# wizzard0/llama2.ts

Measured on AMD Instinct MI355X. Metric: decode tokens/sec + achieved HBM GB/s (% peak), 1 GPU, higher is better.
Workload: dtype f64; 1 GPU; llama2_7b batch-1 greedy decode, 49 tokens from BOS (-t 0 -s 1 -n 49); parallelism=single

## Files before the change

### include/llama2_hip.h

```cpp
#ifndef LLAMA2_HIP_H
#define LLAMA2_HIP_H
#include <stddef.h>
#include <stdint.h>

#ifdef __cplusplus
extern "C" {
#endif

#define L2_ABI_VERSION 5

enum {
  L2_OK = 0,
  L2_E_ARG = -1,
  L2_E_CONFIG = -2,
  L2_E_HIP = -3,
  L2_E_STATE = -4,
  L2_E_NOGPU = -5,
  L2_E_COMM = -6
};

enum {
  L2_T_TOKEN_EMBEDDING = 0,
  L2_T_RMS_ATT = 1,
  L2_T_WQ = 2,
// ... 17 lines not shown
};

enum {
  L2_OPT_EXACT_ATTENTION = 1,
  L2_OPT_USE_GRAPH = 2,
  L2_OPT_KEEP_STATE = 3,
  L2_OPT_PACKED_MIB = 4,
  L2_OPT_WEIGHT_MIB = 5,
  L2_OPT_SAMPLED_TOKENS = 6,
  L2_OPT_SAMPLED_SERIAL = 7,
  L2_OPT_AQL_QUEUE = 8,
  L2_OPT_PREFILL_F32_MFMA = 9,
  L2_OPT_CHECK_POS = 10,
  L2_OPT_SEQS = 11,
  L2_OPT_BATCH_SAMPLED_TOKENS = 12,
  L2_OPT_BATCH_SAMPLED_SERIAL = 13
};

typedef struct l2_ctx l2_ctx;

int l2_abi_version(void);
int l2_device_count(void);
const char* l2_last_error(void);

int l2_create(const int32_t cfg[7], int device, l2_ctx** out);
void l2_destroy(l2_ctx* ctx);

enum { L2_F_GQA = 1, L2_F_GENERATE_ROPE = 2 };
int l2_create_ex(const int32_t cfg[7], int device, unsigned flags, l2_ctx** out);

int l2_tp_unique_id(void* id_out_128);
// ... 63 lines not shown
```

### llama2.ts_amd/csrc/attention.hip.h

```cpp
#pragma once
#include "kernels.hip.h"

namespace l2k {

struct AttnArgs {
  Mut<const float> q;
  Mut<const float> kc;
  Mut<const float> vc;
  Mut<float> att;
  Mut<float> xb;
  const int* tokpos;
  Mut<double> part;
  unsigned* counter;
  int dim, head_size, seq_len, n_heads, nsplit;
  int kv_dim, kv_mul;
  double inv_sqrt_hs;
  int exact;
  int pos_plus1;
  const unsigned long long* gran;
  unsigned* gran_ep;
  int fused_four_waves;
  int* herr;
  unsigned long long wait_ticks;
  unsigned long long* gout;
  const unsigned* gout_ep;
  unsigned long long* dbg;
};

__device__ __forceinline__ void attn_out(const AttnArgs& a, size_t idx, float v, unsigned otag) {
  if (a.gout) granule_store(a.gout + idx, v, otag);
  a.xb.st(idx, v);
}

template <int N>
__device__ __forceinline__ void granules_wait(const unsigned long long* const (&g)[N], float (&v)[N], unsigned tag, int* herr, unsigned long long wait_ticks, unsigned* dead) {
  unsigned spins = 0;
  unsigned long long t0 = 0;
  for (;;) {
    unsigned long long x[N];
#pragma unroll
// ... 77 lines not shown
  if (FUSED) {
    const unsigned tag = ftag = ld_word(const_cast<const unsigned*>(a.gran_ep) + h) + 1u;
    const unsigned long long* gq = a.gran + (size_t)h * hs + cc4;
    const bool need_k = own_pos && wave == NW - 1 && lane < hs, need_v = own_pos && tid < hs;
    const unsigned long long* const gp[7] = {gq, gq + 1, gq + 2, gq + 3,
        need_k ? a.gran + (size_t)h * hs + lane : gq, need_k ? a.gran + (size_t)a.dim + (size_t)hk * hs + lane : gq,
        need_v ? a.gran + (size_t)a.dim + a.kv_dim + (size_t)hk * hs + tid : gq};
    float gvals[7];
    granules_wait<7>(gp, gvals, tag, a.herr, a.wait_ticks, a.gran_ep + a.n_heads);
    STAMP(6);
    q4.x = gvals[0]; q4.y = gvals[1]; q4.z = gvals[2]; q4.w = gvals[3];
    gk_q = need_k ? gvals[4] : 0.0f; gk_k = need_k ? gvals[5] : 0.0f; gv = need_v ? gvals[6] : 0.0f;
  }
  const double q0 = cl ? (double)q4.x : 0.0, q1 = cl ? (double)q4.y : 0.0, q2 = cl ? (double)q4.z : 0.0, q3 = cl ? (double)q4.w : 0.0;
  const double rsq = a.inv_sqrt_hs;
  const unsigned otag = a.gout ? __hip_atomic_load(a.gout_ep, __ATOMIC_RELAXED, __HIP_MEMORY_SCOPE_AGENT) + 1u : 0u;
  double* Pw = P + (size_t)wave * NT * ATT_PS;
  STAMP(1);

  auto score_round = [&](const f4 (&buf)[NT], int rd) {
#pragma unroll
    for (int j = 0; j < NT; ++j) {
      const double s = (q0 * (double)buf[j].x + q1 * (double)buf[j].y) + (q2 * (double)buf[j].z + q3 * (double)buf[j].w);
      Pw[j * ATT_PS + lane] = s;
    }
    __builtin_amdgcn_wave_barrier();
#pragma unroll
    for (int dd = lane; dd < NT * RPT; dd += 64) {
      const int rr = dd / NT, j = dd % NT;
      const int tr = ((rd * NT + j) * NW + wave) * RPT + rr;
      const double* pp = Pw + j * ATT_PS + rr * LR;
// ... 214 lines not shown
  }
  attn_tile_dispatch<LR, 8, NT, true>(at, smem, h, sp, pos);
}

template <int XV, int R, int LR, int NW, int NT>
__global__ void __launch_bounds__(512) attn_wo_kernel(const AttnArgs at, const PhaseArgs wo, const int nattn) {
  extern __shared__ __attribute__((aligned(16))) char smem[];
  if ((int)blockIdx.x >= nattn) { phase_small_body<MODE_WO, XV, R, true>(wo, smem, (int)blockIdx.x - nattn, (int)gridDim.x - nattn); return; }
  if (NW * 64 < 512 && (int)threadIdx.x >= NW * 64) return;
  int sp = 0, h = (int)blockIdx.x;
  while (h >= at.n_heads) { h -= at.n_heads; ++sp; }
  const int pos = at.tokpos[1];
  attn_tile_dispatch<LR, NW, NT>(at, smem, h, sp, pos);
}

template <int LR, int NW, int NT>
__global__ void __launch_bounds__(64 * NW) attn_tile_kernel(const AttnArgs a) {
  extern __shared__ __attribute__((aligned(16))) char smem[];
  asm volatile("" ::"s"(a.q.addr()), "s"(a.kc.addr()), "s"(a.vc.addr()), "s"(a.att.addr()), "s"(a.xb.addr()), "s"(a.tokpos), "s"(a.part.addr()), "s"(a.counter));
  const int pos = a.tokpos[1];
  asm volatile("" ::"s"(a.dim), "s"(a.head_size), "s"(a.seq_len), "s"(a.n_heads), "s"(a.nsplit), "s"(a.kv_dim), "s"(a.kv_mul), "s"(a.inv_sqrt_hs), "s"(a.gout), "s"(a.gout_ep));
  attn_tile_dispatch<LR, NW, NT>(a, smem, blockIdx.x, blockIdx.y, pos);
}

template <int LR, int NW, int NT>
__global__ void __launch_bounds__(64 * NW) pf_attn_tile_kernel(const AttnArgs a, int pos0) {
  extern __shared__ __attribute__((aligned(16))) char smem[];
  AttnArgs b = a;
  const int p = blockIdx.y;
  b.q = a.q + (size_t)p * a.dim;
// ... 79 lines not shown
```

### llama2.ts_amd/csrc/attention_inst.hip.h

```cpp
#pragma once
#include "attention.hip.h"

#ifndef L2_ATTN_INST
#define L2_ATTN_INST extern
#endif

namespace l2k {
#define L2_AT_INST(LR, NW, NT) \
  L2_ATTN_INST template __global__ void attn_tile_kernel<LR, NW, NT>(const AttnArgs); \
  L2_ATTN_INST template __global__ void pf_attn_tile_kernel<LR, NW, NT>(const AttnArgs, int); \
  L2_ATTN_INST template __global__ void bt_attn_tile_kernel<LR, NW, NT>(const AttnArgs, const AttnRows);
L2_AT_INST(4, 4, 16) L2_AT_INST(8, 4, 16) L2_AT_INST(16, 4, 16) L2_AT_INST(32, 8, 8) L2_AT_INST(64, 4, 16)
#undef L2_AT_INST
L2_ATTN_INST template __global__ void qkv_attn_small_kernel<2, 16, 8>(const PhaseArgs, const AttnArgs, const int);
L2_ATTN_INST template __global__ void qkv_attn_small_kernel<3, 16, 8>(const PhaseArgs, const AttnArgs, const int);
L2_ATTN_INST template __global__ void qkv_attn_small_kernel<4, 16, 8>(const PhaseArgs, const AttnArgs, const int);
L2_ATTN_INST template __global__ void attn_wo_kernel<2, 2, 32, 8, 8>(const AttnArgs, const PhaseArgs, const int);
L2_ATTN_INST template __global__ void attn_wo_kernel<4, 2, 32, 8, 8>(const AttnArgs, const PhaseArgs, const int);
L2_ATTN_INST template __global__ void attn_wo_kernel<8, 2, 32, 8, 8>(const AttnArgs, const PhaseArgs, const int);
}
```

### llama2.ts_amd/csrc/ctx.hip.h

```cpp
#pragma once

static thread_local char g_err[512] = "";

static int fail(int code, const char* fmt, ...) {
  va_list ap;
  va_start(ap, fmt);
  vsnprintf(g_err, sizeof(g_err), fmt, ap);
  va_end(ap);
  return code;
}

#define HIPCHK(expr)                                                                              \
  do {                                                                                            \
    hipError_t e_ = (expr);                                                                       \
    if (e_ != hipSuccess) return fail(L2_E_HIP, "%s failed: %s (%s:%d)", #expr, hipGetErrorString(e_), __FILE__, __LINE__); \
  } while (0)

typedef struct { char internal[128]; } nccl_uid;
typedef void* nccl_comm;
struct Rccl {
  void* so = nullptr;
  int (*GetUniqueId)(nccl_uid*) = nullptr;
  int (*CommInitRank)(nccl_comm*, int, nccl_uid, int) = nullptr;
  int (*CommDestroy)(nccl_comm) = nullptr;
// ... 98 lines not shown
  int samp_mode = 0;
  std::shared_ptr<LoopGroup> loop;
  double* loop_tmp = nullptr;
  bool tp_path = false;
  bool p2p = false;
  void* p2p_base = nullptr;
  unsigned long long* p2p_epoch = nullptr;
  int* p2p_err = nullptr;
  int* p2p_err_dev = nullptr;
  P2PPeers p2p_peers = {};
  std::vector<void*> p2p_opened;
  bool p2p_peers_ready = false;
  unsigned long long* awo_gran = nullptr;
  unsigned* awo_ep = nullptr;
  int opt_awo = 1;
  TpPush* tp_push = nullptr;
  int opt_push = 1;
  bool rccl_graph = false;
  unsigned long long p2p_wait_ticks = 3000000000ull;
  int p2p_fenced = 0;
  bool solo = false;
  bool p2p_synced = false;
  bool broken = false;

  float* w[L2_T_COUNT] = {};
  size_t layer_elems[L2_T_COUNT] = {};
  int layers_of[L2_T_COUNT] = {};
  std::vector<uint8_t> uploaded[L2_T_COUNT];

  float *x = nullptr, *xb = nullptr, *xb2 = nullptr, *hb = nullptr, *hb2 = nullptr, *q = nullptr, *k = nullptr,
// ... 135 lines not shown
```

### llama2.ts_amd/csrc/kernels.hip.h

```cpp
#pragma once
#include <hip/hip_runtime.h>
#include <stdint.h>
#include <type_traits>

namespace l2k {

typedef float f4 __attribute__((ext_vector_type(4)));

enum { MODE_QKV = 0, MODE_WO = 1, MODE_W13 = 2, MODE_W2 = 3, MODE_CLS = 4 };

enum { CTR_STRIDE = 32 };

#ifdef L2_STAMPS
#define L2_NSTAMP 12
struct Stamps {
  unsigned long long t[L2_NSTAMP];
  unsigned long long* dst;
  unsigned long long* wg;
  unsigned long long rt0;
  __device__ __forceinline__ Stamps(unsigned long long* dbg, unsigned long long* dbg_wg = nullptr, int force_sel = -2, bool last_wave = false) {
    wg = (dbg_wg && threadIdx.x == (last_wave ? blockDim.x - 64 : 0) && blockIdx.y == 0 && blockIdx.x < 1024) ? dbg_wg + 2 * blockIdx.x : nullptr;
    rt0 = __builtin_readcyclecounter();
    asm volatile("s_memrealtime %0\n\ts_waitcnt lgkmcnt(0)" : "=s"(rt0));
#pragma unroll
// ... 100 lines not shown
  const struct TpPush* push;
  double inv_n;
  int rot;
  const float* wp;
  unsigned long long* amax;
  unsigned long long* gran;
  const unsigned* gran_ep;
  unsigned gran_hmagic;
  int* gin_herr;
  int* tok_out;
#ifdef L2_STAMPS
  unsigned long long* dbg;
  unsigned long long* dbg_wg;
#endif
};
static_assert(sizeof(void*) != 8 || sizeof(PhaseArgs) <= 224 + 16, "PhaseArgs: keep the kernel-argument block within four 64-byte lines");

struct TpPush { unsigned long long* gin[8]; const unsigned long long* epoch; int G, rank, n, solo; };

typedef unsigned u32x4 __attribute__((ext_vector_type(4)));
__device__ __forceinline__ void tp_push_store(unsigned long long* slot, double v, unsigned tag) {
  const unsigned long long b = (unsigned long long)__double_as_longlong(v);
  const u32x4 w = {(unsigned)b, tag, (unsigned)(b >> 32), tag};
  asm volatile("global_store_dwordx4 %0, %1, off sc0 sc1\n\ts_nop 1" ::"v"(slot), "v"(w) : "memory");
}
struct PushCtx { unsigned long long* gin = nullptr; int G = 0, rank = 0, n = 0, solo = 0; unsigned e = 0; };
__device__ __forceinline__ PushCtx tp_push_ctx(const TpPush* p, int lane) {
  PushCtx c;
  c.G = __builtin_amdgcn_readfirstlane(p->G); c.rank = __builtin_amdgcn_readfirstlane(p->rank);
  c.n = __builtin_amdgcn_readfirstlane(p->n); c.solo = __builtin_amdgcn_readfirstlane(p->solo);
  c.gin = p->gin[c.solo ? c.rank : min(lane, c.G - 1)];
// ... 910 lines not shown
```

### llama2.ts_amd/csrc/launch.hip.h

```cpp
#pragma once

struct Geo { int R, U, pre, nwaves, grid; bool vec; };

struct GeoKnobs { int n_cus, tune_U, tune_nwaves, tune_gridcap; };
static GeoKnobs geo_knobs(const l2_ctx* c) { return {c->n_cus, c->tune_U, c->tune_nwaves, c->tune_gridcap}; }

static Geo pick_geo_pure(const GeoKnobs& kb, int mode, int rows, int n) {
  Geo g;
  g.vec = (n % 4) == 0;
  const int n4 = n / 4;
  const int pair = (mode == MODE_W13) ? 2 : 1;
  g.R = 2;
  int U = 2;
  if (n4 > 128 && n4 <= 256) U = 4;
  if (mode == MODE_CLS && n4 > 128 && n4 <= 192) U = 3;
  if (kb.tune_U == 2 || kb.tune_U == 4 || (kb.tune_U == 3 && mode == MODE_CLS && n4 > 128 && n4 <= 192)) U = kb.tune_U;
  g.U = U;
  const int groups = (rows * pair + g.R - 1) / g.R;
  g.nwaves = groups >= 512 ? 4 : (groups >= 256 ? 2 : 1);
  if (kb.tune_nwaves == 1 || kb.tune_nwaves == 2 || kb.tune_nwaves == 4) g.nwaves = kb.tune_nwaves;
  if (mode == MODE_QKV && U == 4) g.nwaves = 4;
  const int cpi = 64 * U, npad4 = ((n4 + cpi - 1) / cpi) * cpi, nth = 64 * g.nwaves;
  g.pre = (npad4 <= nth) ? 1 : (npad4 <= 4 * nth ? 4 : 12);
  int grid = (groups + g.nwaves - 1) / g.nwaves;
// ... 52 lines not shown
    if (!name || aql_record(m->aql, m->aql_rec, name, g, b, (unsigned)lds, buf, off)) m->aql_rec_failed = true;
    return;
  }
  hipLaunchKernelGGL(kernel, grid, block, lds, st, a...);
}

static void pollute_behind(const l2_ctx* c, hipStream_t st) {
  PolluteArgs p;
  memset(&p, 0, sizeof(p));
  int nb = 0;
  auto add = [&](const void* b, size_t bytes) { if (b && bytes && nb < 20) { p.buf[nb] = (const float*)b; p.bytes[nb] = (unsigned)(bytes > 16384 ? 16384 : bytes); ++nb; } };
  add(c->x, (size_t)c->d * 4); add(c->xn, (size_t)c->d * 4); add(c->xb, (size_t)c->d_loc * 4); add(c->xb2, (size_t)c->d * 4);
  add(c->hb, (size_t)c->h_loc * 4); add(c->hb2, (size_t)c->h_loc * 4); add(c->q, (size_t)c->d_loc * 4); add(c->k, (size_t)c->kvd_loc * 4); add(c->v, (size_t)c->kvd_loc * 4);
  add(c->logits_loc, (size_t)c->V_loc * 4); add(c->amax, 8 * 16 * 8); add(c->attn_counter, (size_t)c->H_loc * CTR_STRIDE * 4);
  add(c->attn_part, (size_t)c->H_loc * 8 * (((size_t)c->hs + 2 + 15) & ~(size_t)15) * 8); add(c->gran, ((size_t)c->d_loc + 2 * (size_t)c->kvd_loc) * 8);
  add(c->gran_ep, (size_t)c->H_loc * 4 + 16); add(c->tokpos, 16); add(c->d_tokens, (size_t)c->S * 4); add(c->att, (size_t)c->H_loc * c->S * 4);
  p.nb = nb; p.kc = c->kc; p.vc = c->vc; p.tokpos = c->tokpos; p.sink = c->pollute_sink; p.L = c->L; p.S = c->S; p.kvd = c->kvd_loc;
  l2_launch_one(c, l1_pollute_kernel, dim3(c->n_cus * 4), dim3(256), 0, st, p);
}

template <class K, class A>
static void launch_probed(const l2_ctx* c, K kernel, dim3 grid, dim3 block, size_t lds, hipStream_t st, const A& a, bool probe) {
  l2_ctx* m = const_cast<l2_ctx*>(c);
  if (probe && m->probe_on && m->probe_used + 2 <= m->probe.size()) {
    hipEvent_t e0 = m->probe[m->probe_used], e1 = m->probe[m->probe_used + 1];
    m->probe_used += 2;
    hipExtLaunchKernelGGL(kernel, grid, block, lds, st, e0, e1, 0, a);
  } else {
    l2_launch(c, kernel, grid, block, lds, st, a);
  }
}
// ... 214 lines not shown
  PhaseArgs wo = wo_in;
  wo.gran = c->awo_gran; wo.gran_ep = c->awo_ep; wo.gin_herr = c->h_herr_dev;
  const int nattn = c->H_loc * at.nsplit, xv = (c->d_loc / 4 + 63) / 64;
  const int groups = (wo.rows + 1) / 2;
  int nwo = c->n_cus - nattn;
  if (nwo < c->n_cus / 2) nwo = c->n_cus / 2;
  if (nwo > groups) nwo = groups;
  const size_t lds_a = attn_tile_lds(c->S, at.nsplit, 8, 8), lds_w = (size_t)xv * 64 * 16, lds = lds_a > lds_w ? lds_a : lds_w;
  const dim3 grid(nattn + nwo), block(512);
#define L2_AWO(XVV) do { hipError_t e_ = lds_opt_in(&attn_wo_kernel<XVV, 2, 32, 8, 8>, lds); if (e_ != hipSuccess) return e_; \
                         l2_launch(c, attn_wo_kernel<XVV, 2, 32, 8, 8>, grid, block, lds, st, at, wo, nattn); } while (0)
  if (xv == 2) L2_AWO(2); else if (xv == 4) L2_AWO(4); else L2_AWO(8);
#undef L2_AWO
  return hipGetLastError();
}
```

### llama2.ts_amd/csrc/llama2_hip.hip

```cpp
#include "../../include/llama2_hip.h"

#include <dlfcn.h>
#include <hip/hip_runtime.h>
#include <hip/hip_ext.h>
#include <math.h>
#include <stdarg.h>
#include <stdio.h>
#include <stdlib.h>
#include <string.h>
#include <unistd.h>

#include <chrono>
#include <condition_variable>
#include <map>
#include <memory>
#include <mutex>
#include <string>
#include <type_traits>
#include <algorithm>
#include <vector>

#include "kernels.hip.h"
#include "attention_inst.hip.h"
#include "prefill.hip.h"
// ... 24 lines not shown
    if (c->aql_greedy[i]) { aql_program_free(c->aql_greedy[i]); c->aql_greedy[i] = nullptr; }
    if (c->aql_step[i]) { aql_program_free(c->aql_step[i]); c->aql_step[i] = nullptr; }
    if (i == 0 && c->aql_last) { aql_program_free(c->aql_last); c->aql_last = nullptr; }
    for (int m = 0; m < 4; ++m) if (c->aql_sample[i][m]) { aql_program_free(c->aql_sample[i][m]); c->aql_sample[i][m] = nullptr; }
  }
  if (c->aql) aql_reset(c->aql);
  for (int i = 0; i < NLEV; ++i) {
    if (c->g_step[i]) { hipGraphExecDestroy(c->g_step[i]); c->g_step[i] = nullptr; }
    if (c->g_greedy[i]) { hipGraphExecDestroy(c->g_greedy[i]); c->g_greedy[i] = nullptr; }
    for (int m = 0; m < 4; ++m) if (c->g_sample[i][m]) { hipGraphExecDestroy(c->g_sample[i][m]); c->g_sample[i][m] = nullptr; }
  }
}

static const int kSplitLevels[NLEV] = {1, 1, 8};
static bool fused_shape_ok(const l2_ctx* c);
static int split_level(const l2_ctx* c, int pos) {
  if (c->attn_splits_forced > 0 || c->opt_exact) return 0;
  const bool fusable = fused_shape_ok(c);
  int unsplit_to = (c->split_rows_set || !fusable) ? c->split_rows : 256;
  if (fusable && unsplit_to > 256) unsplit_to = 256;
  const int rows = pos + 1;
  if (rows > unsplit_to) return 2;
  return (fusable && rows > c->fuse_min_rows) ? 1 : 0;
}
static int splits_of(const l2_ctx* c, int level) { return c->attn_splits_forced > 0 ? c->attn_splits_forced : kSplitLevels[level]; }
static void set_level(l2_ctx* c, int level) {
  c->cur_splits = splits_of(c, level);
  c->cur_fused = level == 1 || (c->opt_fuse_splits && !c->opt_exact && fused_shape_ok(c));
}

extern "C" void l2_destroy(l2_ctx* c) {
  if (!c) return;
  hipSetDevice(c->device);
  if (c->stream) hipStreamSynchronize(c->stream);
  destroy_graphs(c);
  batch_free(c);
  if (c->aql) { aql_destroy(c->aql); c->aql = nullptr; }
  if (c->comm && g_rccl.CommDestroy) g_rccl.CommDestroy(c->comm);
  if (c->loop_tmp) hipFree(c->loop_tmp);
  for (void* m : c->p2p_opened) hipIpcCloseMemHandle(m);
  if (c->p2p_base) hipFree(c->p2p_base);
  if (c->p2p_epoch) hipFree(c->p2p_epoch);
  if (c->tp_push) hipFree(c->tp_push);
// ... 73 lines not shown
  c->tune_gridcap = dev_int("L2_TUNE_GRIDCAP", 0);
  c->tune_rot = dev_int("L2_TUNE_ROT", 5);
  c->opt_packed = dev_int("L2_PACKED", 1);
  c->opt_one_copy = dev_int("L2_ONE_COPY", 1);
  c->opt_graph = env_int("L2_USE_GRAPH", (G == 1 && !hook_int("L2_TP_FORCE_COMM")) ? 1 : 0);
  c->profile_sync = dev_int("L2_PROFILE_SYNC", 0);
  c->opt_aql = env_int("L2_AQL", 1);
  c->opt_pollute = hook_int("L2_DEBUG_POLLUTE");
  c->debug_fail_aql = hook_int("L2_DEBUG_FAIL_AQL_RUN");
  c->opt_pos_check = env_int("L2_CHECK_POS", 0);
  { const int f = dev_int("L2_AQL_FENCE", -1);
    c->aql_fence = dev_int("L2_AQL_ACQ", f < 0 ? 0 : f) + 4 * dev_int("L2_AQL_REL", f < 0 ? 1 : f) + 16 * dev_int("L2_AQL_TOKACQ", f < 0 ? 1 : 0); }
  c->p2p_fenced = env_int("L2_TP_FENCED", 0) ? 1 : 0;
  c->opt_push = dev_int("L2_TP_PUSH", 1) && !c->p2p_fenced;
  c->opt_awo = dev_int("L2_TP_ATTN_WO", 1);
  { const int ws = env_int("L2_TP_WAIT_S", 30); c->p2p_wait_ticks = (unsigned long long)(ws > 0 ? ws : 30) * 100000000ull; }

#define CK(expr) do { hipError_t e_ = (expr); if (e_ != hipSuccess) { int rc_ = fail(L2_E_HIP, "%s failed: %s", #expr, hipGetErrorString(e_)); l2_destroy(c); return rc_; } } while (0)
  CK(hipStreamCreateWithFlags(&c->stream, hipStreamNonBlocking));
  CK(hipEventCreate(&c->ev0));
  CK(hipEventCreate(&c->ev1));
  for (int k = 0; k < L2_T_COUNT; ++k) {
    const Slice s = tensor_slice(c, k);
    c->layers_of[k] = is_layered(k) ? L : 1;
    c->layer_elems[k] = s.rows * s.cols;
    if (k == L2_T_WCLS && c->shared) {
      if (G == 1) { c->w[k] = c->w[L2_T_TOKEN_EMBEDDING]; c->uploaded[k].assign(1, 0); continue; }
      c->w[k] = c->w[L2_T_TOKEN_EMBEDDING] + (size_t)rank * c->V_loc * d;
      c->uploaded[k].assign(1, 0);
      continue;
    }
    CK(hipMalloc(&c->w[k], c->layer_elems[k] * c->layers_of[k] * sizeof(float)));
    c->uploaded[k].assign(c->layers_of[k], 0);
  }
  const size_t dl = c->d_loc, kvl = c->kvd_loc, kv = (size_t)L * S * kvl;
  CK(hipMalloc(&c->x, d * 4)); CK(hipMalloc(&c->xn, d * 4));
  CK(hipMalloc(&c->xb, dl * 4)); CK(hipMalloc(&c->xb2, d * 4));
  CK(hipMalloc(&c->hb, c->h_loc * 4)); CK(hipMalloc(&c->hb2, c->h_loc * 4));
  CK(hipMalloc(&c->q, dl * 4)); CK(hipMalloc(&c->k, kvl * 4)); CK(hipMalloc(&c->v, kvl * 4));
  CK(hipMalloc(&c->att, (size_t)c->H_loc * S * 4));
  c->tp_path = G > 1 || hook_int("L2_TP_FORCE_COMM");
  if (c->tp_path) CK(hipExtMallocWithFlags((void**)&c->logits, (size_t)V * 4, hipDeviceMallocUncached));
  else CK(hipMalloc(&c->logits, (size_t)V * 4));
  if (c->tp_path) { CK(hipMalloc(&c->logits_loc, (size_t)c->V_loc * 4)); CK(hipMalloc(&c->partial, (size_t)d * 8)); }
  if (c->tp_path) {
    CK(hipMalloc(&c->awo_gran, (size_t)c->d_loc * 8)); CK(hipMemsetAsync(c->awo_gran, 0, (size_t)c->d_loc * 8, c->stream));
    CK(hipMalloc(&c->awo_ep, 16)); CK(hipMemsetAsync(c->awo_ep, 0, 16, c->stream));
  }
  else c->logits_loc = c->logits;
  CK(hipMalloc(&c->kc, kv * 4)); CK(hipMalloc(&c->vc, kv * 4));
  CK(hipMemsetAsync(c->kc, 0, kv * 4, c->stream)); CK(hipMemsetAsync(c->vc, 0, kv * 4, c->stream));
  float* zero[] = {c->x, c->xn, c->xb, c->xb2, c->hb, c->hb2, c->q, c->k, c->v};
  const size_t zn[] = {(size_t)d, (size_t)d, dl, (size_t)d, (size_t)c->h_loc, (size_t)c->h_loc, dl, kvl, kvl};
  for (int i = 0; i < 9; ++i) CK(hipMemsetAsync(zero[i], 0, zn[i] * 4, c->stream));
  CK(hipMemsetAsync(c->att, 0, (size_t)c->H_loc * S * 4, c->stream));
  CK(hipMemsetAsync(c->logits, 0, (size_t)V * 4, c->stream));
  c->attn_splits_forced = dev_int("L2_ATTN_SPLITS", 0);
  c->split_rows = dev_int("L2_ATTN_SPLIT_ROWS", 144);
  c->split_rows_set = dev_int("L2_ATTN_SPLIT_ROWS", -1) >= 0;
  c->small_max = dev_int("L2_SMALL_MAX", 8 << 20);
  c->n_cus = prop.multiProcessorCount > 0 ? prop.multiProcessorCount : 256;
  c->pf3 = dev_int("L2_PF3", 1);
  c->pf_attn = dev_int("L2_PF_ATTN", 1);
  if (c->attn_splits_forced > 64) c->attn_splits_forced = 64;
// ... 361 lines not shown
  return L2_OK;
}

static bool greedy_folds(const l2_ctx* c) { return !c->tp_path && c->amax && c->d % 4 == 0 && c->h % 4 == 0; }
static int enqueue_forward_impl(l2_ctx* c, hipStream_t st, bool to_host, int fold = 0) {
  auto greedy = [&](PhaseArgs& a) { if (fold == 2) { a.amax = c->amax; a.tok_out = c->d_tokens; } };
  for (int l = 0; l < c->L; ++l) {
    PhaseArgs a = qkv_args(c, l);
    if (l == 0) greedy(a);
    if (fused_qkv_attn_ok(c)) {
      LCHK(launch_qkv_attn(c, a, l, st));
    } else {
      LCHK(launch_phase<MODE_QKV>(c, a, st));
      if (attn_wo_ok(c)) {
        LCHK(launch_attn_wo(c, l, wo_args(c, l), st));
      } else {
        LCHK(launch_attn(c, l, st));
        a = wo_args(c, l);
        if (l == 0) greedy(a);
        LCHK(launch_phase<MODE_WO>(c, a, st));
      }
    }
    if (fused_qkv_attn_ok(c)) {
      a = wo_args(c, l);
      if (l == 0) greedy(a);
      LCHK(launch_phase<MODE_WO>(c, a, st));
    }
    if (c->p2p) {
      const int rc_ = p2p_reduce(c, st, (l == 0) ? c->w[L2_T_TOKEN_EMBEDDING] : nullptr, c->opt_keep_state ? c->xb2 : nullptr, attn_wo_ok(c) ? c->awo_ep : nullptr);
      if (rc_) return rc_;
// ... 204 lines not shown
  if (timed && ms) *ms = (float)(us * 1e-3);
  c->ran_forward = true;
  return check_p2p(c);
}

extern "C" int l2_forward(l2_ctx* c, int token, int pos, float* logits_out) {
  if (!c) return fail(L2_E_ARG, "null context");
  if (pos < 0 || pos >= c->S) return fail(L2_E_ARG, "pos %d outside [0, seq_len=%d)", pos, c->S);
  if (token < 0 || token >= c->V) return fail(L2_E_ARG, "token %d outside [0, vocab_size=%d)", token, c->V);
  if (c->opt_pos_check && pos != 0 && pos > c->next_pos)
    return fail(L2_E_STATE, "L2_CHECK_POS: pos %d skips ahead of the sequence (cache rows 0 .. %d have been written)", pos, c->next_pos - 1);
  int rc = ensure_ready(c);
  if (rc) return rc;
  HIPCHK(hipSetDevice(c->device));
  c->next_pos = pos + 1;
  c->h_tokpos[0] = token; c->h_tokpos[1] = pos; c->h_tokpos[2] = 0; c->h_tokpos[3] = 0;
  const int lvl = split_level(c, pos);
  set_level(c, lvl);
  if (aql_usable(c) && c->opt_zero_copy && !c->tp_path && (c->aql || !aql_open(c)) && !aql_record_level(c, lvl, enqueue_forward_call, &c->aql_step[lvl])) {
    HIPCHK(hipStreamSynchronize(c->stream));
    if (aql_run_c(c, 1, &c->aql_step[lvl], nullptr)) return aql_give_up(c);
    c->ran_forward = true;
    rc = check_p2p(c);
    if (rc) return rc;
    if (logits_out) memcpy(logits_out, c->h_logits, (size_t)c->V * 4);
    return L2_OK;
  }
  set_level(c, lvl);
  int (*enq)(l2_ctx*, hipStream_t) = c->tp_path ? enqueue_forward_host : enqueue_forward_call;
  if (c->tp_path) HIPCHK(hipMemcpyAsync(c->tokpos, c->h_tokpos, 4 * sizeof(int), hipMemcpyHostToDevice, c->stream));
  if (c->opt_graph) {
    if (!c->g_step[lvl]) { rc = capture(c, enq, &c->g_step[lvl]); if (rc && rc != L2_RUN_EAGER) return rc; }
  }
// ... 14 lines not shown
}

extern "C" float* l2_logits_host(l2_ctx* c) { return c ? c->h_logits : nullptr; }

#include "prefill_host.hip.h"
#include "batch_host.hip.h"

static int run_greedy(l2_ctx* c, int first_token, int pos0, int steps, bool timed, float* ms) {
  if (!c) return fail(L2_E_ARG, "null context");
  if (steps < 0 || pos0 < 0 || pos0 + steps > c->S) return fail(L2_E_ARG, "pos0 %d + steps %d exceeds seq_len %d", pos0, steps, c->S);
  if (first_token < 0 || first_token >= c->V) return fail(L2_E_ARG, "token out of range");
  int rc = ensure_ready(c);
  if (rc) return rc;
  HIPCHK(hipSetDevice(c->device));
  if (pos0 + steps > c->next_pos || pos0 == 0) c->next_pos = pos0 + steps;
  c->h_tokpos[0] = first_token; c->h_tokpos[1] = pos0; c->h_tokpos[2] = 0; c->h_tokpos[3] = 0;
  HIPCHK(hipMemcpyAsync(c->tokpos, c->h_tokpos, 4 * sizeof(int), hipMemcpyHostToDevice, c->stream));
  HIPCHK(hipMemsetAsync(c->amax, 0, 8 * 16 * 8, c->stream));
  if (aql_usable(c)) {
    const int rc_a = run_greedy_aql(c, pos0, steps, timed, ms);
    if (rc_a != L2_RUN_EAGER) return rc_a;
  }
  if (c->opt_graph) {
    for (int s = 0; s < steps; ++s) {
      const int lvl = split_level(c, pos0 + s);
      if (!c->g_greedy[lvl]) { set_level(c, lvl); rc = capture(c, enqueue_greedy, &c->g_greedy[lvl]); if (rc == L2_RUN_EAGER) break; if (rc) return rc; }
    }
  }
  if (timed) HIPCHK(hipEventRecord(c->ev0, c->stream));
  for (int s = 0; s < steps; ++s) {
    const int lvl = split_level(c, pos0 + s);
// ... 20 lines not shown
  if (!(temperature == temperature) || !(topp == topp)) return fail(L2_E_ARG, "temperature / topp is NaN");
  int rc = ensure_ready(c);
  if (rc) return rc;
  if (steps < 0 || pos0 < 0 || pos0 + steps > c->S) return fail(L2_E_ARG, "positions %d..%d outside [0, %d)", pos0, pos0 + steps, c->S);
  if (first_token < 0 || first_token >= c->V) return fail(L2_E_ARG, "token %d outside [0, %d)", first_token, c->V);
  if (steps == 0) return L2_OK;
  HIPCHK(hipSetDevice(c->device));
  if (!c->samp.V) {
    if (c->V > l2s::MAX_VOCAB) return fail(L2_E_CONFIG, "device sampler supports vocabularies up to %d", (int)l2s::MAX_VOCAB);
    HIPCHK(l2s::create(&c->samp, c->V));
  }
  const double params[2] = {temperature, topp};
  c->samp_mode = (topp <= 0 || topp >= 1) ? 0 : 1;
  c->samp_amax = !c->tp_path && temperature > 0 && c->amax && !c->samp.serial;
  HIPCHK(hipMemsetAsync(c->amax, 0, 8 * 16 * 8, c->stream));
  c->h_tokpos[0] = first_token; c->h_tokpos[1] = pos0; c->h_tokpos[2] = 0; c->h_tokpos[3] = 0;
  HIPCHK(hipMemcpyAsync(c->tokpos, c->h_tokpos, 4 * sizeof(int), hipMemcpyHostToDevice, c->stream));
  HIPCHK(hipMemcpyAsync(c->samp.params, params, sizeof(params), hipMemcpyHostToDevice, c->stream));
  HIPCHK(hipMemcpyAsync(c->samp.rng, rng_state, sizeof(uint64_t), hipMemcpyHostToDevice, c->stream));
  HIPCHK(hipStreamSynchronize(c->stream));
  if (aql_usable(c) && (c->aql || !aql_open(c))) {
    const int mode = c->samp_mode + (c->samp_amax ? 2 : 0);
    bool ok = true;
    std::vector<AqlProgram*> per(steps);
    for (int s = 0; s < steps && ok; ++s) {
      const int lvl = split_level(c, pos0 + s);
      if (aql_record_level(c, lvl, enqueue_sample, &c->aql_sample[lvl][mode])) ok = false;
      else per[s] = c->aql_sample[lvl][mode];
    }
    if (ok) {
      if (aql_run_c(c, steps, per.data(), nullptr)) return aql_give_up(c);
// ... 86 lines not shown
extern "C" int l2_set_option(l2_ctx* c, int key, int value) {
  if (!c) return fail(L2_E_ARG, "null context");
  switch (key) {
    case L2_OPT_EXACT_ATTENTION:
      if (c->opt_exact != !!value) {
        c->opt_exact = !!value;
        destroy_graphs(c);
      }
      return L2_OK;
    case L2_OPT_USE_GRAPH: c->opt_graph = !!value; return L2_OK;
    case L2_OPT_KEEP_STATE: if (c->opt_keep_state != !!value) { c->opt_keep_state = !!value; destroy_graphs(c); } return L2_OK;
    case L2_OPT_AQL_QUEUE: c->opt_aql = !!value; if (value) c->aql_tried = false; return L2_OK;
    case L2_OPT_PREFILL_F32_MFMA: c->opt_pf_f32 = !!value; return L2_OK;
    case L2_OPT_CHECK_POS: c->opt_pos_check = !!value; return L2_OK;
    case L2_OPT_PACKED_MIB: case L2_OPT_WEIGHT_MIB: case L2_OPT_SAMPLED_TOKENS: case L2_OPT_SAMPLED_SERIAL: case L2_OPT_SEQS:
    case L2_OPT_BATCH_SAMPLED_TOKENS: case L2_OPT_BATCH_SAMPLED_SERIAL:
      return fail(L2_E_ARG, "option %d is read-only", key);
    default: return fail(L2_E_ARG, "unknown option %d", key);
  }
}

extern "C" int l2_get_option(l2_ctx* c, int key, int* value) {
  if (!c || !value) return fail(L2_E_ARG, "null argument");
  switch (key) {
    case L2_OPT_EXACT_ATTENTION: *value = c->opt_exact; return L2_OK;
    case L2_OPT_USE_GRAPH: *value = c->opt_graph; return L2_OK;
    case L2_OPT_KEEP_STATE: *value = c->opt_keep_state; return L2_OK;
    case L2_OPT_AQL_QUEUE: *value = aql_usable(c) ? 1 : 0; return L2_OK;
    case L2_OPT_PREFILL_F32_MFMA: *value = c->opt_pf_f32; return L2_OK;
    case L2_OPT_CHECK_POS: *value = c->opt_pos_check; return L2_OK;
    case L2_OPT_SEQS: *value = c->bt ? c->bt->n_seqs : 0; return L2_OK;
    case L2_OPT_BATCH_SAMPLED_TOKENS: case L2_OPT_BATCH_SAMPLED_SERIAL: {
      const unsigned long long v = c->bt ? c->bt->smp_stats[key == L2_OPT_BATCH_SAMPLED_SERIAL ? 1 : 0] : 0;
      *value = v > 0x7fffffffull ? 0x7fffffff : (int)v;
      return L2_OK;
    }
    case L2_OPT_PACKED_MIB: {
      size_t floats = 0;
      if (c->packed_valid) for (int m = 0; m < 5; ++m) if (c->packed[m].buf) floats += c->packed[m].layer_elems * (size_t)(m == MODE_CLS ? 1 : c->L);
      *value = (int)(floats * sizeof(float) >> 20);
      return L2_OK;
    }
    case L2_OPT_WEIGHT_MIB: {
      size_t floats = 0;
      for (int k = 0; k < L2_T_COUNT; ++k) if (c->w[k] && !(k == L2_T_WCLS && c->shared)) floats += c->layer_elems[k] * (size_t)c->layers_of[k];
      for (int m = 0; m < 5; ++m) if (c->packed[m].buf) floats += c->packed[m].layer_elems * (size_t)(m == MODE_CLS ? 1 : c->L);
// ... 27 lines not shown
```

### llama2.ts_amd/runtime.py

```python
import ctypes as C
import os
import struct

import numpy as np

_HERE = os.path.dirname(os.path.abspath(__file__))
LIB_PATH = os.environ.get("L2_LIB_PATH") or os.path.join(_HERE, "lib", "libllama2hip.so")

T_TOKEN_EMBEDDING, T_RMS_ATT, T_WQ, T_WK, T_WV, T_WO, T_RMS_FFN, T_W1, T_W2, T_W3, T_RMS_FINAL, \
    T_FREQ_REAL, T_FREQ_IMAG, T_WCLS = range(14)
TENSOR_NAMES = ["token_embedding_table", "rms_att_weight", "wq", "wk", "wv", "wo", "rms_ffn_weight", "w1", "w2",
                "w3", "rms_final_weight", "freq_cis_real", "freq_cis_imag", "wcls"]
S_X, S_XB, S_XB2, S_HB, S_HB2, S_Q, S_K, S_V, S_ATT, S_LOGITS, S_KEY_CACHE, S_VALUE_CACHE = range(12)
STATE_IDS = dict(x=S_X, xb=S_XB, xb2=S_XB2, hb=S_HB, hb2=S_HB2, q=S_Q, k=S_K, v=S_V, att=S_ATT, logits=S_LOGITS,
                 key_cache=S_KEY_CACHE, value_cache=S_VALUE_CACHE)
OPT_EXACT_ATTENTION, OPT_USE_GRAPH, OPT_KEEP_STATE, OPT_PACKED_MIB, OPT_WEIGHT_MIB, OPT_SAMPLED_TOKENS, OPT_SAMPLED_SERIAL, OPT_AQL_QUEUE, OPT_PREFILL_F32_MFMA, OPT_CHECK_POS = 1, 2, 3, 4, 5, 6, 7, 8, 9, 10
OPT_SEQS = 11
OPT_BATCH_SAMPLED_TOKENS, OPT_BATCH_SAMPLED_SERIAL = 12, 13
F_GQA, F_GENERATE_ROPE = 1, 2
TP_SOLO_ID = b"L2-SOLO-SHARD-TIMING"

ABI_SYMBOLS = ["l2_abi_version", "l2_device_count", "l2_last_error", "l2_create", "l2_destroy", "l2_tp_unique_id",
               "l2_create_tp", "l2_upload", "l2_synth_fill", "l2_read_tensor", "l2_forward", "l2_logits_host",
               "l2_decode_greedy", "l2_decode_sample", "l2_debug_running_sums", "l2_read_state", "l2_set_option", "l2_get_option", "l2_timer_start",
               "l2_timer_stop", "l2_bench_gemv", "l2_bench_decode", "l2_load_checkpoint", "l2_get_header", "l2_prefill", "l2_bench_dominant_in_situ", "l2_tp_mode", "l2_create_ex", "l2_bench_tokens", "l2_dispatch_reason",
               "l2_seq_reserve", "l2_seq_prefill", "l2_forward_batch", "l2_decode_greedy_batch", "l2_read_seq_cache",
               "l2_decode_sample_batch", "l2_seq_prefill_batch", "l2_step_batch", "l2_seq_score_batch", "l2_step_batch_logprobs",
               "l2_seq_fork"]


class L2Error(RuntimeError):
    def __init__(self, code, text):
        super().__init__("libllama2hip: %s (code %d)" % (text, code))
# ... 441 lines not shown
```

Baseline: 233.9 tokens/s.

## Fuse attention with streaming WO GEMV in one single-GPU kernel

Adds a single-GPU kernel that runs the attention heads and the WO projection in one launch. Attention blocks publish their output through tagged granules, and extra WO blocks prefetch their weight chunks with nontemporal loads while they wait on those granules. This removes a kernel boundary per layer and overlaps WO weight streaming with attention. In exchange it depends on spin-waiting across blocks in the same grid, so it assumes enough CUs for co-residency and adds a per-run nonce to tag data.

```diff
diff --git a/include/llama2_hip.h b/include/llama2_hip.h
--- a/include/llama2_hip.h
+++ b/include/llama2_hip.h
@@ -55,7 +55,8 @@
   L2_OPT_CHECK_POS = 10,
   L2_OPT_SEQS = 11,
   L2_OPT_BATCH_SAMPLED_TOKENS = 12,
-  L2_OPT_BATCH_SAMPLED_SERIAL = 13
+  L2_OPT_BATCH_SAMPLED_SERIAL = 13,
+  L2_OPT_ATTN_WO_STREAM = 14
 };
 
 typedef struct l2_ctx l2_ctx;
diff --git a/llama2.ts_amd/csrc/attention.hip.h b/llama2.ts_amd/csrc/attention.hip.h
--- a/llama2.ts_amd/csrc/attention.hip.h
+++ b/llama2.ts_amd/csrc/attention.hip.h
@@ -24,6 +24,7 @@
   unsigned long long wait_ticks;
   unsigned long long* gout;
   const unsigned* gout_ep;
+  unsigned gout_tag;
   unsigned long long* dbg;
 };
 
@@ -131,7 +132,7 @@
   }
   const double q0 = cl ? (double)q4.x : 0.0, q1 = cl ? (double)q4.y : 0.0, q2 = cl ? (double)q4.z : 0.0, q3 = cl ? (double)q4.w : 0.0;
   const double rsq = a.inv_sqrt_hs;
-  const unsigned otag = a.gout ? __hip_atomic_load(a.gout_ep, __ATOMIC_RELAXED, __HIP_MEMORY_SCOPE_AGENT) + 1u : 0u;
+  const unsigned otag = a.gout ? (a.gout_tag ? a.gout_tag : __hip_atomic_load(a.gout_ep, __ATOMIC_RELAXED, __HIP_MEMORY_SCOPE_AGENT) + 1u) : 0u;
   double* Pw = P + (size_t)wave * NT * ATT_PS;
   STAMP(1);
 
@@ -376,6 +377,97 @@
   attn_tile_dispatch<LR, NW, NT>(at, smem, h, sp, pos);
 }
 
+__device__ __forceinline__ unsigned attn_wo_stream_tag(int nonce, int pos, int layer, int n_layers) {
+  return 0x80000000u | (((unsigned)nonce & 0x7ffu) << 20) | (((unsigned)pos * (unsigned)n_layers + (unsigned)layer) & 0xfffffu);
+}
+
+constexpr int AWOS_WAVES = 10;
+
+template <int NCH>
+__device__ __forceinline__ void wo_stream_body(const PhaseArgs& a, char* smem, const int vblock, const unsigned tag, int token, const int pos,
+                                               int* herr, const unsigned long long wait_ticks) {
+  constexpr int R = 2, U = 2;
+  constexpr int CH = NCH * 16;
+  constexpr int NU = (CH + 63) / 64;
+  f4* xs4 = reinterpret_cast<f4*>(smem);
+  const int tid = threadIdx.x, lane = tid & 63, wave = __builtin_amdgcn_readfirstlane(tid >> 6);
+  const int groups = (a.rows + R - 1) / R;
+  const int place = vblock * AWOS_WAVES + wave;
+  const bool have = place < groups;
+  const int pl = have ? place : groups - 1;
+  const f4* base = reinterpret_cast<const f4*>(a.wp) + (size_t)pl * (R * U * 64) + lane;
+  const size_t cstride = (size_t)groups * (R * U * 64);
+  f4 w[NCH][R][U];
+  auto issue = [&](int ci) {
+#pragma unroll
+    for (int u = 0; u < U; ++u)
+#pragma unroll
+      for (int r = 0; r < R; ++r) w[ci][r][u] = __builtin_nontemporal_load(base + cstride * ci + (r * U + u) * 64);
+  };
+#pragma unroll
+  for (int ci = 0; ci < NCH; ++ci) issue(ci);
+  if (a.emb && a.tok_out) {
+    const int step = a.tokpos[2];
+    if (step > 0) token = a.tok_out[step - 1];
+    if (vblock == 0 && tid < 8) a.amax[(size_t)tid * 16] = 0ull;
+  }
+  const EpiPre pre = epi_prefetch<MODE_WO, R>(a, pl, lane, token, pos);
+  if (wave < 8) {
+    f4 xr[NU];
+    granules_gather_f4<NU>(a.gran + (size_t)wave * (CH * 4), CH * 4, lane, tag, xr, herr, wait_ticks, 1, const_cast<unsigned*>(a.gran_ep) + 1);
+#pragma unroll
+    for (int u = 0; u < NU; ++u)
+      if (u * 64 + lane < CH) xs4[wave * CH + u * 64 + lane] = xr[u];
+  }
+#ifdef L2_STAMPS
+  if (a.dbg_wg && tid == 0 && blockIdx.x < 1024) { unsigned long long t; asm volatile("s_memrealtime %0\n\ts_waitcnt lgkmcnt(0)" : "=s"(t)); a.dbg_wg[2048 + 2 * blockIdx.x] = t; }
+#endif
+  __syncthreads();
+  double acc[R];
+#pragma unroll
+  for (int r = 0; r < R; ++r) acc[r] = 0.0;
+#pragma unroll
+  for (int ci = 0; ci < NCH; ++ci) {
+#pragma unroll
+    for (int u = 0; u < U; ++u) {
+      const f4 xv = xs4[ci * (64 * U) + u * 64 + lane];
+      const double x0 = xv.x, x1 = xv.y, x2 = xv.z, x3 = xv.w;
+#pragma unroll
+      for (int r = 0; r < R; ++r) {
+        acc[r] += (double)w[ci][r][u].x * x0;
+        acc[r] += (double)w[ci][r][u].y * x1;
+        acc[r] += (double)w[ci][r][u].z * x2;
+        acc[r] += (double)w[ci][r][u].w * x3;
+      }
+    }
+  }
+  wave_sum2(acc[0], acc[R - 1]);
+  unsigned long long nobest = 0;
+  if (have) finish_group<MODE_WO, R, true>(a, place, acc, lane, token, pos, pre, nobest);
+}
+
+template <int NCH>
+__global__ void __launch_bounds__(64 * AWOS_WAVES) attn_wo_stream_kernel(const AttnArgs at, const PhaseArgs wo, const int nattn, const int layer, const int n_layers) {
+  extern __shared__ __attribute__((aligned(16))) char smem[];
+#define L2_PIN4(x0, x1, x2, x3) asm volatile("" ::"s"(x0), "s"(x1), "s"(x2), "s"(x3))
+  L2_PIN4(wo.wp, wo.tokpos, wo.emb, wo.res.addr()); L2_PIN4(wo.out.addr(), wo.aux.addr(), wo.gran, wo.gran_ep); L2_PIN4(wo.rows, wo.dim, wo.tok_out, wo.amax);
+  L2_PIN4(wo.partial, wo.push, wo.gin_herr, nattn); L2_PIN4(at.q.addr(), at.kc.addr(), at.vc.addr(), at.att.addr()); L2_PIN4(at.xb.addr(), at.tokpos, at.gout, at.dim);
+  L2_PIN4(at.head_size, at.seq_len, at.n_heads, at.nsplit); L2_PIN4(at.kv_dim, at.kv_mul, at.inv_sqrt_hs, at.exact); L2_PIN4(at.wait_ticks, layer, n_layers, at.dbg);
+#undef L2_PIN4
+#ifdef L2_STAMPS
+  Stamps st_(nullptr, wo.dbg_wg);
+#endif
+  const int token = wo.tokpos[0], pos = wo.tokpos[1], nonce = wo.tokpos[3];
+  const unsigned tag = attn_wo_stream_tag(nonce, pos, layer, n_layers);
+  if ((int)blockIdx.x >= nattn) { wo_stream_body<NCH>(wo, smem, (int)blockIdx.x - nattn, tag, token, pos, wo.gin_herr, at.wait_ticks); return; }
+  if ((int)threadIdx.x >= 512) return;
+  int sp = 0, h = (int)blockIdx.x;
+  while (h >= at.n_heads) { h -= at.n_heads; ++sp; }
+  AttnArgs b = at;
+  b.gout_tag = tag;
+  attn_tile_dispatch<32, 8, 8>(b, smem, h, sp, pos);
+}
+
 template <int LR, int NW, int NT>
 __global__ void __launch_bounds__(64 * NW) attn_tile_kernel(const AttnArgs a) {
   extern __shared__ __attribute__((aligned(16))) char smem[];
diff --git a/llama2.ts_amd/csrc/attention_inst.hip.h b/llama2.ts_amd/csrc/attention_inst.hip.h
--- a/llama2.ts_amd/csrc/attention_inst.hip.h
+++ b/llama2.ts_amd/csrc/attention_inst.hip.h
@@ -18,4 +18,7 @@
 L2_ATTN_INST template __global__ void attn_wo_kernel<2, 2, 32, 8, 8>(const AttnArgs, const PhaseArgs, const int);
 L2_ATTN_INST template __global__ void attn_wo_kernel<4, 2, 32, 8, 8>(const AttnArgs, const PhaseArgs, const int);
 L2_ATTN_INST template __global__ void attn_wo_kernel<8, 2, 32, 8, 8>(const AttnArgs, const PhaseArgs, const int);
+L2_ATTN_INST template __global__ void attn_wo_stream_kernel<2>(const AttnArgs, const PhaseArgs, const int, const int, const int);
+L2_ATTN_INST template __global__ void attn_wo_stream_kernel<4>(const AttnArgs, const PhaseArgs, const int, const int, const int);
+L2_ATTN_INST template __global__ void attn_wo_stream_kernel<8>(const AttnArgs, const PhaseArgs, const int, const int, const int);
 }
diff --git a/llama2.ts_amd/csrc/ctx.hip.h b/llama2.ts_amd/csrc/ctx.hip.h
--- a/llama2.ts_amd/csrc/ctx.hip.h
+++ b/llama2.ts_amd/csrc/ctx.hip.h
@@ -136,6 +136,10 @@
   unsigned long long* awo_gran = nullptr;
   unsigned* awo_ep = nullptr;
   int opt_awo = 1;
+  int opt_awo_stream = 1;
+  bool cur_awo_stream = false;
+  bool last_awo_stream = false;
+  unsigned run_nonce = 0;
   TpPush* tp_push = nullptr;
   int opt_push = 1;
   bool rccl_graph = false;
diff --git a/llama2.ts_amd/csrc/kernels.hip.h b/llama2.ts_amd/csrc/kernels.hip.h
--- a/llama2.ts_amd/csrc/kernels.hip.h
+++ b/llama2.ts_amd/csrc/kernels.hip.h
@@ -138,7 +138,9 @@
   unsigned long long* dbg_wg;
 #endif
 };
+#ifndef L2_STAMPS
 static_assert(sizeof(void*) != 8 || sizeof(PhaseArgs) <= 224 + 16, "PhaseArgs: keep the kernel-argument block within four 64-byte lines");
+#endif
 
 struct TpPush { unsigned long long* gin[8]; const unsigned long long* epoch; int G, rank, n, solo; };
 
diff --git a/llama2.ts_amd/csrc/launch.hip.h b/llama2.ts_amd/csrc/launch.hip.h
--- a/llama2.ts_amd/csrc/launch.hip.h
+++ b/llama2.ts_amd/csrc/launch.hip.h
@@ -90,7 +90,7 @@
   add(c->hb, (size_t)c->h_loc * 4); add(c->hb2, (size_t)c->h_loc * 4); add(c->q, (size_t)c->d_loc * 4); add(c->k, (size_t)c->kvd_loc * 4); add(c->v, (size_t)c->kvd_loc * 4);
   add(c->logits_loc, (size_t)c->V_loc * 4); add(c->amax, 8 * 16 * 8); add(c->attn_counter, (size_t)c->H_loc * CTR_STRIDE * 4);
   add(c->attn_part, (size_t)c->H_loc * 8 * (((size_t)c->hs + 2 + 15) & ~(size_t)15) * 8); add(c->gran, ((size_t)c->d_loc + 2 * (size_t)c->kvd_loc) * 8);
-  add(c->gran_ep, (size_t)c->H_loc * 4 + 16); add(c->tokpos, 16); add(c->d_tokens, (size_t)c->S * 4); add(c->att, (size_t)c->H_loc * c->S * 4);
+  add(c->gran_ep, (size_t)c->H_loc * 4 + 16); add(c->awo_gran, (size_t)c->d_loc * 8); add(c->tokpos, 16); add(c->d_tokens, (size_t)c->S * 4); add(c->att, (size_t)c->H_loc * c->S * 4);
   p.nb = nb; p.kc = c->kc; p.vc = c->vc; p.tokpos = c->tokpos; p.sink = c->pollute_sink; p.L = c->L; p.S = c->S; p.kvd = c->kvd_loc;
   l2_launch_one(c, l1_pollute_kernel, dim3(c->n_cus * 4), dim3(256), 0, st, p);
 }
@@ -335,3 +335,43 @@
 #undef L2_AWO
   return hipGetLastError();
 }
+
+static bool attn_wo_stream_shape_ok(const l2_ctx* c) {
+  if (!c->opt_awo_stream || c->tp_path || c->G != 1 || !c->awo_gran || !c->awo_ep || !c->h_herr_dev || !attn_vec(c)) return false;
+  if (c->hs != 128 || c->KVH <= 0 || c->d_loc != c->d || !(c->d == 1024 || c->d == 2048 || c->d == 4096)) return false;
+  if (use_small(c, MODE_WO, c->d, c->d)) return false;
+  const l2_ctx::Packed& p = c->packed[MODE_WO];
+  if (!c->packed_valid || !p.buf || p.U != 2) return false;
+  const Geo g = pick_geo(c, MODE_WO, c->d, c->d, c->d);
+  if (!(g.vec && g.U == 2 && g.nwaves == p.nwaves && g.grid == p.grid)) return false;
+  const int groups = c->d / 2;
+  if (groups > p.grid * p.nwaves) return false;
+  if ((long long)c->S * c->L > 0xfffff) return false;
+  if (c->H + (groups + AWOS_WAVES - 1) / AWOS_WAVES > c->n_cus) return false;
+  return (size_t)attn_tile_lds(c->S, 1, 8, 8) <= 160 * 1024;
+}
+static bool attn_wo_stream_ok(const l2_ctx* c) {
+  return c->cur_awo_stream && c->cur_splits == 1 && !c->opt_exact && c->attn_splits_forced <= 0 && attn_wo_stream_shape_ok(c);
+}
+
+static hipError_t launch_attn_wo_stream(const l2_ctx* c, int l, const PhaseArgs& wo_in, hipStream_t st) {
+  AttnArgs at;
+  fill_attn_args(c, l, at);
+  at.gout = c->awo_gran; at.wait_ticks = 200000000ull;
+  PhaseArgs wo = wo_in;
+  wo.gran = c->awo_gran; wo.gran_ep = c->awo_ep; wo.gin_herr = c->h_herr_dev;
+  if (!wo.wp) return hipErrorInvalidValue;
+#ifdef L2_STAMPS
+  wo.dbg_wg = c->dbg + 66 * 108 + (size_t)(g_stamp_slot % 64) * 2048; g_stamp_slot += 2;
+  wo.dbg = nullptr;
+#endif
+  const int nattn = c->H * at.nsplit, nch = c->d / 512;
+  const int nwo = (c->d / 2 + AWOS_WAVES - 1) / AWOS_WAVES;
+  const size_t lds_a = attn_tile_lds(c->S, at.nsplit, 8, 8), lds_w = (size_t)c->d * 4, lds = lds_a > lds_w ? lds_a : lds_w;
+  const dim3 grid(nattn + nwo), block(64 * AWOS_WAVES);
+#define L2_AWOS(NCH) do { hipError_t e_ = lds_opt_in(&attn_wo_stream_kernel<NCH>, lds); if (e_ != hipSuccess) return e_; \
+                          l2_launch(c, attn_wo_stream_kernel<NCH>, grid, block, lds, st, at, wo, nattn, l, c->L); } while (0)
+  if (nch == 2) L2_AWOS(2); else if (nch == 4) L2_AWOS(4); else L2_AWOS(8);
+#undef L2_AWOS
+  return hipGetLastError();
+}
diff --git a/llama2.ts_amd/csrc/llama2_hip.hip b/llama2.ts_amd/csrc/llama2_hip.hip
--- a/llama2.ts_amd/csrc/llama2_hip.hip
+++ b/llama2.ts_amd/csrc/llama2_hip.hip
@@ -62,19 +62,29 @@
 
 static const int kSplitLevels[NLEV] = {1, 1, 8};
 static bool fused_shape_ok(const l2_ctx* c);
+static bool attn_wo_stream_shape_ok(const l2_ctx* c);
+static const int kAwoStreamRows = 256;
 static int split_level(const l2_ctx* c, int pos) {
   if (c->attn_splits_forced > 0 || c->opt_exact) return 0;
   const bool fusable = fused_shape_ok(c);
-  int unsplit_to = (c->split_rows_set || !fusable) ? c->split_rows : 256;
+  const bool awos = !fusable && attn_wo_stream_shape_ok(c);
+  int unsplit_to = c->split_rows_set ? c->split_rows : (fusable ? 256 : (awos ? kAwoStreamRows : c->split_rows));
   if (fusable && unsplit_to > 256) unsplit_to = 256;
   const int rows = pos + 1;
   if (rows > unsplit_to) return 2;
+  if (awos) return 1;
   return (fusable && rows > c->fuse_min_rows) ? 1 : 0;
+}
+static void note_awo_stream(l2_ctx* c, int pos0, int steps) {
+  c->last_awo_stream = false;
+  if (!attn_wo_stream_shape_ok(c)) return;
+  for (int s = 0; s < steps && !c->last_awo_stream; ++s) c->last_awo_stream = split_level(c, pos0 + s) == 1;
 }
 static int splits_of(const l2_ctx* c, int level) { return c->attn_splits_forced > 0 ? c->attn_splits_forced : kSplitLevels[level]; }
 static void set_level(l2_ctx* c, int level) {
   c->cur_splits = splits_of(c, level);
   c->cur_fused = level == 1 || (c->opt_fuse_splits && !c->opt_exact && fused_shape_ok(c));
+  c->cur_awo_stream = level == 1;
 }
 
 extern "C" void l2_destroy(l2_ctx* c) {
@@ -178,6 +188,7 @@
   c->p2p_fenced = env_int("L2_TP_FENCED", 0) ? 1 : 0;
   c->opt_push = dev_int("L2_TP_PUSH", 1) && !c->p2p_fenced;
   c->opt_awo = dev_int("L2_TP_ATTN_WO", 1);
+  c->opt_awo_stream = dev_int("L2_ATTN_WO_STREAM", 1);
   { const int ws = env_int("L2_TP_WAIT_S", 30); c->p2p_wait_ticks = (unsigned long long)(ws > 0 ? ws : 30) * 100000000ull; }
 
 #define CK(expr) do { hipError_t e_ = (expr); if (e_ != hipSuccess) { int rc_ = fail(L2_E_HIP, "%s failed: %s", #expr, hipGetErrorString(e_)); l2_destroy(c); return rc_; } } while (0)
@@ -207,11 +218,9 @@
   if (c->tp_path) CK(hipExtMallocWithFlags((void**)&c->logits, (size_t)V * 4, hipDeviceMallocUncached));
   else CK(hipMalloc(&c->logits, (size_t)V * 4));
   if (c->tp_path) { CK(hipMalloc(&c->logits_loc, (size_t)c->V_loc * 4)); CK(hipMalloc(&c->partial, (size_t)d * 8)); }
-  if (c->tp_path) {
-    CK(hipMalloc(&c->awo_gran, (size_t)c->d_loc * 8)); CK(hipMemsetAsync(c->awo_gran, 0, (size_t)c->d_loc * 8, c->stream));
-    CK(hipMalloc(&c->awo_ep, 16)); CK(hipMemsetAsync(c->awo_ep, 0, 16, c->stream));
-  }
-  else c->logits_loc = c->logits;
+  CK(hipMalloc(&c->awo_gran, (size_t)c->d_loc * 8)); CK(hipMemsetAsync(c->awo_gran, 0, (size_t)c->d_loc * 8, c->stream));
+  CK(hipMalloc(&c->awo_ep, 16)); CK(hipMemsetAsync(c->awo_ep, 0, 16, c->stream));
+  if (!c->tp_path) c->logits_loc = c->logits;
   CK(hipMalloc(&c->kc, kv * 4)); CK(hipMalloc(&c->vc, kv * 4));
   CK(hipMemsetAsync(c->kc, 0, kv * 4, c->stream)); CK(hipMemsetAsync(c->vc, 0, kv * 4, c->stream));
   float* zero[] = {c->x, c->xn, c->xb, c->xb2, c->hb, c->hb2, c->q, c->k, c->v};
@@ -603,6 +612,10 @@
       LCHK(launch_phase<MODE_QKV>(c, a, st));
       if (attn_wo_ok(c)) {
         LCHK(launch_attn_wo(c, l, wo_args(c, l), st));
+      } else if (attn_wo_stream_ok(c)) {
+        a = wo_args(c, l);
+        if (l == 0) greedy(a);
+        LCHK(launch_attn_wo_stream(c, l, a, st));
       } else {
         LCHK(launch_attn(c, l, st));
         a = wo_args(c, l);
@@ -837,9 +850,10 @@
   if (rc) return rc;
   HIPCHK(hipSetDevice(c->device));
   c->next_pos = pos + 1;
-  c->h_tokpos[0] = token; c->h_tokpos[1] = pos; c->h_tokpos[2] = 0; c->h_tokpos[3] = 0;
+  c->h_tokpos[0] = token; c->h_tokpos[1] = pos; c->h_tokpos[2] = 0; c->h_tokpos[3] = (int)(++c->run_nonce & 0x7ffu);
   const int lvl = split_level(c, pos);
   set_level(c, lvl);
+  note_awo_stream(c, pos, 1);
   if (aql_usable(c) && c->opt_zero_copy && !c->tp_path && (c->aql || !aql_open(c)) && !aql_record_level(c, lvl, enqueue_forward_call, &c->aql_step[lvl])) {
     HIPCHK(hipStreamSynchronize(c->stream));
     if (aql_run_c(c, 1, &c->aql_step[lvl], nullptr)) return aql_give_up(c);
@@ -884,7 +898,8 @@
   if (rc) return rc;
   HIPCHK(hipSetDevice(c->device));
   if (pos0 + steps > c->next_pos || pos0 == 0) c->next_pos = pos0 + steps;
-  c->h_tokpos[0] = first_token; c->h_tokpos[1] = pos0; c->h_tokpos[2] = 0; c->h_tokpos[3] = 0;
+  c->h_tokpos[0] = first_token; c->h_tokpos[1] = pos0; c->h_tokpos[2] = 0; c->h_tokpos[3] = (int)(++c->run_nonce & 0x7ffu);
+  note_awo_stream(c, pos0, steps);
   HIPCHK(hipMemcpyAsync(c->tokpos, c->h_tokpos, 4 * sizeof(int), hipMemcpyHostToDevice, c->stream));
   HIPCHK(hipMemsetAsync(c->amax, 0, 8 * 16 * 8, c->stream));
   if (aql_usable(c)) {
@@ -935,7 +950,8 @@
   c->samp_mode = (topp <= 0 || topp >= 1) ? 0 : 1;
   c->samp_amax = !c->tp_path && temperature > 0 && c->amax && !c->samp.serial;
   HIPCHK(hipMemsetAsync(c->amax, 0, 8 * 16 * 8, c->stream));
-  c->h_tokpos[0] = first_token; c->h_tokpos[1] = pos0; c->h_tokpos[2] = 0; c->h_tokpos[3] = 0;
+  c->h_tokpos[0] = first_token; c->h_tokpos[1] = pos0; c->h_tokpos[2] = 0; c->h_tokpos[3] = (int)(++c->run_nonce & 0x7ffu);
+  note_awo_stream(c, pos0, steps);
   HIPCHK(hipMemcpyAsync(c->tokpos, c->h_tokpos, 4 * sizeof(int), hipMemcpyHostToDevice, c->stream));
   HIPCHK(hipMemcpyAsync(c->samp.params, params, sizeof(params), hipMemcpyHostToDevice, c->stream));
   HIPCHK(hipMemcpyAsync(c->samp.rng, rng_state, sizeof(uint64_t), hipMemcpyHostToDevice, c->stream));
@@ -1052,7 +1068,7 @@
     case L2_OPT_PREFILL_F32_MFMA: c->opt_pf_f32 = !!value; return L2_OK;
     case L2_OPT_CHECK_POS: c->opt_pos_check = !!value; return L2_OK;
     case L2_OPT_PACKED_MIB: case L2_OPT_WEIGHT_MIB: case L2_OPT_SAMPLED_TOKENS: case L2_OPT_SAMPLED_SERIAL: case L2_OPT_SEQS:
-    case L2_OPT_BATCH_SAMPLED_TOKENS: case L2_OPT_BATCH_SAMPLED_SERIAL:
+    case L2_OPT_BATCH_SAMPLED_TOKENS: case L2_OPT_BATCH_SAMPLED_SERIAL: case L2_OPT_ATTN_WO_STREAM:
       return fail(L2_E_ARG, "option %d is read-only", key);
     default: return fail(L2_E_ARG, "unknown option %d", key);
   }
@@ -1068,6 +1084,7 @@
     case L2_OPT_PREFILL_F32_MFMA: *value = c->opt_pf_f32; return L2_OK;
     case L2_OPT_CHECK_POS: *value = c->opt_pos_check; return L2_OK;
     case L2_OPT_SEQS: *value = c->bt ? c->bt->n_seqs : 0; return L2_OK;
+    case L2_OPT_ATTN_WO_STREAM: *value = c->last_awo_stream ? 1 : 0; return L2_OK;
     case L2_OPT_BATCH_SAMPLED_TOKENS: case L2_OPT_BATCH_SAMPLED_SERIAL: {
       const unsigned long long v = c->bt ? c->bt->smp_stats[key == L2_OPT_BATCH_SAMPLED_SERIAL ? 1 : 0] : 0;
       *value = v > 0x7fffffffull ? 0x7fffffff : (int)v;
diff --git a/llama2.ts_amd/runtime.py b/llama2.ts_amd/runtime.py
--- a/llama2.ts_amd/runtime.py
+++ b/llama2.ts_amd/runtime.py
@@ -17,6 +17,7 @@
 OPT_EXACT_ATTENTION, OPT_USE_GRAPH, OPT_KEEP_STATE, OPT_PACKED_MIB, OPT_WEIGHT_MIB, OPT_SAMPLED_TOKENS, OPT_SAMPLED_SERIAL, OPT_AQL_QUEUE, OPT_PREFILL_F32_MFMA, OPT_CHECK_POS = 1, 2, 3, 4, 5, 6, 7, 8, 9, 10
 OPT_SEQS = 11
 OPT_BATCH_SAMPLED_TOKENS, OPT_BATCH_SAMPLED_SERIAL = 12, 13
+OPT_ATTN_WO_STREAM = 14
 F_GQA, F_GENERATE_ROPE = 1, 2
 TP_SOLO_ID = b"L2-SOLO-SHARD-TIMING"
 
```

Result: faster. 237.1 tokens/s (median of 6 runs) (+1.4%).
